# nonl4331/raytracing-rust

Measured on AMD Instinct MI355X. Metric: Msamples/s on rtweekend1.ssml 1920x1080x1024spp, higher is better.
Workload: dtype f32

## Files before the change

include/rt_hip.h:

```cpp
#ifndef RT_HIP_H
#define RT_HIP_H

#include <stdint.h>

#ifdef __cplusplus
extern "C" {
#endif

#define RT_ABI_VERSION 2u

typedef enum rt_status {
	RT_OK = 0,
	RT_ERR_INVALID_ARGUMENT = -1,
	RT_ERR_NO_DEVICE = -2,
	RT_ERR_HIP = -3,
	RT_ERR_OUT_OF_MEMORY = -4,
	RT_ERR_UNSUPPORTED = -5
} rt_status;

typedef enum rt_texture_type {
	RT_TEX_CHECKERED = 0,
	RT_TEX_SOLID = 1,
	RT_TEX_IMAGE = 2,
	RT_TEX_LERP = 3,
// ... 162 lines not shown
#define RT_DEVICE_NONE (-1)
void rt_scene_destroy(rt_scene *scene);

int rt_scene_create_multi(const rt_scene_desc *desc, const int *devices, uint32_t n_devices, rt_scene **out);
int rt_scene_device_count(const rt_scene *scene, uint32_t *n_devices);
typedef enum rt_gather_mode { RT_GATHER_NONE = 0, RT_GATHER_RCCL = 1, RT_GATHER_PEER = 2, RT_GATHER_PEER_STAGED = 3, RT_GATHER_SAME_DEVICE = 4 } rt_gather_mode;
int rt_scene_gather_info(const rt_scene *scene, int *mode, char *note, uint64_t note_capacity);
int rt_rccl_probe(int *usable, char *note, uint64_t note_capacity);
int rt_scene_auto_sample_split(const rt_scene *scene, const rt_render_opts *opts, uint32_t *split);

int rt_scene_counts(const rt_scene *scene, uint64_t *n_nodes, uint64_t *n_primitives, uint64_t *n_lights);
int rt_scene_get_nodes(const rt_scene *scene, rt_bvh_node *out, uint64_t capacity);
int rt_scene_get_primitive_order(const rt_scene *scene, uint64_t *out, uint64_t capacity);
int rt_scene_get_lights(const rt_scene *scene, uint64_t *out, uint64_t capacity);
int rt_scene_wide_info(const rt_scene *scene, uint64_t *n_wide_nodes, uint32_t *root_ref, uint32_t *stack_depth);
int rt_scene_get_wide_nodes(const rt_scene *scene, void *out, uint64_t capacity_nodes);
int rt_scene_get_leaf_boxes(const rt_scene *scene, float *out, uint64_t capacity_slots);
int rt_scene_get_wide_nodes_compact(const rt_scene *scene, void *out, uint64_t capacity_nodes);
int rt_scene_get_leaf_boxes_compact(const rt_scene *scene, float *out, uint64_t capacity_leaves, uint64_t *n_leaves);

typedef struct rt_sky_info {
	uint32_t res_x, res_y;
	uint32_t guide_k;
	uint32_t inv_res_ok;
	float inv_res_x, inv_res_y;
	uint64_t table_bytes;
} rt_sky_info;
int rt_scene_sky_info(const rt_scene *scene, rt_sky_info *info);
int rt_scene_get_sky_tables(const rt_scene *scene, float *row_cdf, uint64_t capacity_rows, float *marginal_cdf, uint64_t capacity_marginal,
                            uint8_t *guide, uint64_t capacity_guide);

int rt_scene_set_traversal(rt_scene *scene, int mode);
typedef enum rt_tuning_key { RT_TUNE_TRAVERSAL = 0, RT_TUNE_FEATURE_SET = 1, RT_TUNE_SCENE_IN_LDS = 2, RT_TUNE_SCHEDULE = 3, RT_TUNE_WALK = 4,
                             RT_TUNE_STACK_CAP = 5, RT_TUNE_EXCHANGE = 6, RT_TUNE_WHOLE_PIXEL_SHARE = 7 } rt_tuning_key;
int rt_scene_set_tuning(rt_scene *scene, int key, int value);
int rt_plan_work_items(const rt_render_opts *opts, uint32_t split, int share, uint64_t resident_waves, uint32_t *whole_claims,
                       uint64_t *n_items);

int rt_render(rt_scene *scene, const rt_camera *camera, const rt_render_opts *opts, float *out_rgb,
              uint64_t *rays_shot);

int rt_render_device(rt_scene *scene, const rt_camera *camera, const rt_render_opts *opts, float *d_out_rgb,
                     uint64_t *d_rays_shot, void *hip_stream);

int rt_render_output_floats(const rt_render_opts *opts, uint64_t *n_floats);
int rt_shard_pixel_order(const rt_render_opts *opts, uint64_t *out, uint64_t capacity);

typedef struct rt_sampler_progress {
	uint64_t samples_completed;
	uint64_t rays_shot;
	const float *current_image;
	uint64_t n_floats;
} rt_sampler_progress;
typedef int (*rt_presentation_update)(void *data, const rt_sampler_progress *progress, uint64_t samples_done);
int rt_sample_image(rt_scene *scene, const rt_camera *camera, const rt_render_opts *opts, uint64_t batch,
                    rt_presentation_update update, void *data);

int rt_last_kernel_ms(rt_scene *scene, float *ms, uint32_t *n_launches);

typedef struct rt_launch_info {
	int32_t method;
	int32_t pruned;
	int32_t fine;
	int32_t sky_in_lds;
	int32_t scene_in_lds;
	int32_t feature_set;
	uint32_t block_threads;
	uint32_t n_blocks;
	uint32_t blocks_per_cu;
	uint32_t waves_per_simd;
	uint32_t lds_bytes;
	uint32_t n_cus;
	uint32_t sample_split;
	uint32_t whole_claims;
	uint64_t n_items;
	char kernel[160];
} rt_launch_info;
int rt_last_launch_info(const rt_scene *scene, rt_launch_info *out);

int rt_output_rgb8(const float *rgb, uint64_t n_values, float gamma, uint8_t *out);
int rt_output_save(const char *filename, const float *rgb, uint32_t width, uint32_t height, float gamma);

int rt_output_rgb8_device(rt_scene *scene, const float *d_rgb, uint64_t n_values, float gamma, uint8_t *d_out, void *hip_stream);
int rt_render_rgb8(rt_scene *scene, const rt_camera *camera, const rt_render_opts *opts, float gamma, uint8_t *out_rgb8,
                   uint64_t *rays_shot);

int rt_check_hit(rt_scene *scene, const rt_ray_desc *rays, uint64_t n_rays, rt_hit_record *out);
int rt_check_hit_index(rt_scene *scene, const rt_ray_desc *rays, const uint64_t *object_index, uint64_t n_rays,
                       rt_hit_record *out);

typedef struct rt_aov_buffers {
	float *albedo;
	float *normal;
	float *depth;
	float *coverage;
	uint32_t *primitive;
	uint32_t *material;
} rt_aov_buffers;
int rt_render_aov(rt_scene *scene, const rt_camera *camera, const rt_render_opts *opts, const rt_aov_buffers *host_out);
int rt_render_aov_device(rt_scene *scene, const rt_camera *camera, const rt_render_opts *opts, const rt_aov_buffers *device_out,
                         void *hip_stream);

typedef struct rt_aov_chain_opts {
	uint32_t max_chain;
	float fuzz_limit;
	uint32_t reserved[6];
} rt_aov_chain_opts;
typedef struct rt_aov_chain_buffers {
// ... 259 lines not shown
```

raytracing-rust_amd/abi.py:

```python
import ctypes as C

RT_ABI_VERSION = 2
RT_GATHER_NONE, RT_GATHER_RCCL, RT_GATHER_PEER, RT_GATHER_PEER_STAGED, RT_GATHER_SAME_DEVICE = 0, 1, 2, 3, 4

RT_OK = 0
RT_ERR_INVALID_ARGUMENT = -1
RT_ERR_NO_DEVICE = -2
RT_ERR_HIP = -3
RT_ERR_OUT_OF_MEMORY = -4
RT_ERR_UNSUPPORTED = -5

RT_TEX_CHECKERED, RT_TEX_SOLID, RT_TEX_IMAGE, RT_TEX_LERP, RT_TEX_PERLIN = range(5)
RT_MAT_EMIT, RT_MAT_LAMBERTIAN, RT_MAT_TROWBRIDGE_REITZ, RT_MAT_REFLECT, RT_MAT_REFRACT = range(5)
RT_PRIM_SPHERE, RT_PRIM_TRIANGLE, RT_PRIM_MESH_TRIANGLE = range(3)
RT_SPLIT_SAH, RT_SPLIT_MIDDLE, RT_SPLIT_EQUAL_COUNTS = range(3)
RT_METHOD_NAIVE, RT_METHOD_MIS = range(2)
RT_LAYOUT_FRAME, RT_LAYOUT_SHARD = range(2)
RT_TUNE_TRAVERSAL, RT_TUNE_FEATURE_SET, RT_TUNE_SCENE_IN_LDS, RT_TUNE_SCHEDULE, RT_TUNE_WALK, RT_TUNE_STACK_CAP, RT_TUNE_EXCHANGE, RT_TUNE_WHOLE_PIXEL_SHARE = range(8)

NO_INDEX = 0xFFFFFFFFFFFFFFFF
RT_DEVICE_NONE = -1

f32x3 = C.c_float * 3


class TextureDesc(C.Structure):
    _fields_ = [
        ("type", C.c_int32),
        ("colour_one", f32x3),
        ("colour_two", f32x3),
        ("image_rgb", C.POINTER(C.c_float)),
        ("image_width", C.c_uint32),
        ("image_height", C.c_uint32),
        ("perlin_ran_vecs", C.POINTER(C.c_float)),
        ("perlin_perm", C.POINTER(C.c_uint32)),
    ]


class MaterialDesc(C.Structure):
    _fields_ = [
        ("type", C.c_int32),
        ("texture", C.c_uint32),
        ("param", C.c_float),
        ("ior", f32x3),
        ("metallic", C.c_float),
    ]


class _Sphere(C.Structure):
    _fields_ = [("centre", f32x3), ("radius", C.c_float)]

# ... 103 lines not shown
        ("max", f32x3),
        ("children", C.c_int64 * 2),
        ("primitive_offset", C.c_uint64),
        ("number_primitives", C.c_uint64),
    ]


class SamplerProgressC(C.Structure):
    _fields_ = [
        ("samples_completed", C.c_uint64),
        ("rays_shot", C.c_uint64),
        ("current_image", C.POINTER(C.c_float)),
        ("n_floats", C.c_uint64),
    ]


class LaunchInfo(C.Structure):
    _fields_ = [
        ("method", C.c_int32),
        ("pruned", C.c_int32),
        ("fine", C.c_int32),
        ("sky_in_lds", C.c_int32),
        ("scene_in_lds", C.c_int32),
        ("feature_set", C.c_int32),
        ("block_threads", C.c_uint32),
        ("n_blocks", C.c_uint32),
        ("blocks_per_cu", C.c_uint32),
        ("waves_per_simd", C.c_uint32),
        ("lds_bytes", C.c_uint32),
        ("n_cus", C.c_uint32),
        ("sample_split", C.c_uint32),
        ("whole_claims", C.c_uint32),
        ("n_items", C.c_uint64),
        ("kernel", C.c_char * 160),
    ]


class SkyInfo(C.Structure):
    _fields_ = [
        ("res_x", C.c_uint32),
        ("res_y", C.c_uint32),
        ("guide_k", C.c_uint32),
        ("inv_res_ok", C.c_uint32),
        ("inv_res_x", C.c_float),
        ("inv_res_y", C.c_float),
        ("table_bytes", C.c_uint64),
    ]


class AovBuffers(C.Structure):
    _fields_ = [
        ("albedo", C.POINTER(C.c_float)),
        ("normal", C.POINTER(C.c_float)),
        ("depth", C.POINTER(C.c_float)),
        ("coverage", C.POINTER(C.c_float)),
        ("primitive", C.POINTER(C.c_uint32)),
        ("material", C.POINTER(C.c_uint32)),
    ]


AOV_CHANNELS = ("albedo", "normal", "depth", "coverage", "primitive", "material")


class AovChainOpts(C.Structure):
    _fields_ = [
        ("max_chain", C.c_uint32),
# ... 265 lines not shown
        ("sigma_normal", C.c_float),
        ("depth_tolerance", C.c_float),
        ("reserved", C.c_uint32 * 8),
    ]


UPSCALE_INPUTS = ("color", "src_albedo", "src_normal", "src_depth", "dst_albedo", "dst_normal", "dst_depth")
UPSCALE_GUIDES = ("albedo", "normal", "depth")
UPSCALE_OPTIONS = ("sigma_normal", "depth_tolerance")


class UpscaleInputs(C.Structure):
    _fields_ = [(name, C.POINTER(C.c_float)) for name in UPSCALE_INPUTS]


DISPLAY_OPTIONS = tuple(n for n, _ in DisplayOpts._fields_ if n not in ("width", "height", "reserved"))

PresentationUpdate = C.CFUNCTYPE(C.c_int, C.c_void_p, C.POINTER(SamplerProgressC), C.c_uint64)

EXPECTED_SIZES = {
    "rt_texture_desc": (TextureDesc, 64),
    "rt_material_desc": (MaterialDesc, 28),
    "rt_primitive_desc": (PrimitiveDesc, 40),
    "rt_triangle_data": (TriangleData, 72),
    "rt_mesh_desc": (MeshDesc, 32),
    "rt_sky_desc": (SkyDesc, 16),
    "rt_scene_desc": (SceneDesc, 96),
    "rt_camera": (Camera, 48),
    "rt_render_opts": (RenderOpts, 80),
    "rt_hit_record": (HitRecord, 72),
    "rt_ray_desc": (RayDesc, 24),
    "rt_bvh_node": (BvhNode, 56),
    "rt_sampler_progress": (SamplerProgressC, 32),
    "rt_launch_info": (LaunchInfo, 224),
    "rt_sky_info": (SkyInfo, 32),
    "rt_aov_buffers": (AovBuffers, 48),
    "rt_aov_chain_opts": (AovChainOpts, 32),
    "rt_aov_chain_buffers": (AovChainBuffers, 56),
    "rt_matte_opts": (MatteOpts, 32),
    "rt_matte_buffers": (MatteBuffers, 24),
    "rt_ao_opts": (AoOpts, 32),
    "rt_ao_buffers": (AoBuffers, 16),
    "rt_noise_opts": (NoiseOpts, 32),
    "rt_noise_summary": (NoiseSummary, 16),
    "rt_noise_buffers": (NoiseBuffers, 40),
    "rt_noise_result": (NoiseResult, 40),
    "rt_robust_opts": (RobustOpts, 32),
    "rt_robust_buffers": (RobustBuffers, 40),
    "rt_denoise_opts": (DenoiseOpts, 48),
    "rt_denoise_inputs": (DenoiseInputs, 40),
    "rt_temporal_opts": (TemporalOpts, 96),
    "rt_temporal_inputs": (TemporalInputs, 32),
    "rt_display_opts": (DisplayOpts, 104),
    "rt_display_state": (DisplayState, 16),
    "rt_bloom_opts": (BloomOpts, 64),
    "rt_dof_opts": (DofOpts, 64),
    "rt_upscale_opts": (UpscaleOpts, 56),
    "rt_upscale_inputs": (UpscaleInputs, 56),
}

EXPORTED_SYMBOLS = [
    "rt_last_error",
    "rt_abi_version",
    "rt_device_count",
    "rt_render_opts_default",
    "rt_camera_new",
    "rt_scene_create",
# ... 150 lines not shown
```

raytracing-rust_amd/csrc/rt_api.cpp:

```cpp
#include <hip/hip_runtime.h>

#include <cstdio>
#include <cstdlib>
#include <algorithm>
#include <cmath>
#include <cstring>
#include <string>
#include <vector>

#include "../../include/rt_hip.h"
#include "../../include/rt_detmath.h"
#include <dlfcn.h>
#include "rt_api_internal.h"
#include "rt_render.h"

using namespace rt;

thread_local std::string g_error;

constexpr uint32_t kFineAboveTriangles = 4096;
constexpr uint32_t kFineAboveSpheres = 32768;

struct RcclApi {
	void *lib = nullptr;
// ... 607 lines not shown
{
	switch (key) {
	case RT_TUNE_TRAVERSAL:
		return rt_scene_set_traversal(s, value);
	case RT_TUNE_FEATURE_SET:
		if (value < s->min_feature_set || value > 2)
			return fail(RT_ERR_INVALID_ARGUMENT, "feature set must be between the scene's own and 2");
		s->feature_set = value;
		s->feature_set_forced = true;
		return RT_OK;
	case RT_TUNE_SCHEDULE:
		if (value < -1 || value > 1)
			return fail(RT_ERR_INVALID_ARGUMENT, "schedule must be -1, 0 or 1");
		s->schedule_mode = value;
		return RT_OK;
	case RT_TUNE_SCENE_IN_LDS:
		s->scene_lds_allowed = value != 0;
		return RT_OK;
	case RT_TUNE_STACK_CAP:
		if (value < 0 || value > 96)
			return fail(RT_ERR_INVALID_ARGUMENT, "stack cap must be 0 (automatic) or 1..96 entries");
		s->stack_cap_override = (uint32_t)value;
		return RT_OK;
	case RT_TUNE_EXCHANGE:
		if (value < 0 || value > 1)
			return fail(RT_ERR_INVALID_ARGUMENT, "exchange must be 0 (off) or 1 (on where the kernel has it)");
		s->exchange_mode = value;
		return RT_OK;
	case RT_TUNE_WHOLE_PIXEL_SHARE:
		if (value < -1 || value > 16)
			return fail(RT_ERR_INVALID_ARGUMENT, "whole-pixel share must be -1 (automatic) or 0..16 (sixteenths of a shard's tiles)");
		s->whole_share = value;
		return RT_OK;
	case RT_TUNE_WALK:
		if (value < 0 || value > 1)
			return fail(RT_ERR_INVALID_ARGUMENT, "walk must be 0 (automatic) or 1 (two-child walk for every ray)");
		s->dev.narrow_only = (uint32_t)value;
		return RT_OK;
	default:
		return fail(RT_ERR_INVALID_ARGUMENT, "unknown tuning key");
	}
}

int rt_scene_counts(const rt_scene *s, uint64_t *n_nodes, uint64_t *n_primitives, uint64_t *n_lights)
{
	if (!s)
		return fail(RT_ERR_INVALID_ARGUMENT, "null scene");
	if (n_nodes) *n_nodes = s->host.nodes.size();
	if (n_primitives) *n_primitives = s->host.primitive_order.size();
	if (n_lights) *n_lights = s->host.lights.size();
	return RT_OK;
}
int rt_scene_get_nodes(const rt_scene *s, rt_bvh_node *out, uint64_t capacity)
{
	if (!s || !out || capacity < s->host.nodes.size())
		return fail(RT_ERR_INVALID_ARGUMENT, "bad arguments");
	for (size_t i = 0; i < s->host.nodes.size(); ++i) {
		const HostNode &n = s->host.nodes[i];
		std::memcpy(out[i].min, n.min, 12);
		std::memcpy(out[i].max, n.max, 12);
		out[i].children[0] = n.child[0];
		out[i].children[1] = n.child[1];
		out[i].primitive_offset = n.primitive_offset;
		out[i].number_primitives = n.number_primitives;
	}
	return RT_OK;
// ... 183 lines not shown

static void fill_tiling(DevRenderParams &P, const rt_render_opts *o, const ShardGeometry &g)
{
	P.width = (uint32_t)o->width;
	P.height = (uint32_t)o->height;
	P.shard_index = o->shard_index;
	P.shard_count = o->shard_count;
	P.tile_w = g.tile_w;
	P.tile_h = g.tile_h;
	P.tiles_x = g.tiles_x;
	P.tiles_y = g.tiles_y;
	P.n_work = (uint32_t)g.n_work;
}

static uint32_t tiled_order_log2(const rt_render_opts *o, const ShardGeometry &g, uint32_t split)
{
	if (g.tile_w * g.tile_h == 64u && (g.tile_w & (g.tile_w - 1u)) == 0u && o->width < 65536u && o->height < 65536u &&
	    (split & (split - 1u)) == 0u && split <= 64u)
		for (uint32_t lw = 0; lw < 7u; ++lw)
			for (uint32_t ls = 0; ls < 7u; ++ls)
				if ((1u << lw) == g.tile_w && (1u << ls) == split)
					return lw | (ls << 8);
	return 0xFFFFFFFFu;
}

struct RenderLaunchPlan {
	DevRenderParams P;
	DevScene dev;
	bool prune, fine, sky_lds, scene_lds, xchg;
	int feature_set, blocks_per_cu;
	uint32_t block_threads, n_blocks;
	size_t lds_bytes;
	uint32_t split;
};

static int plan_render_launch(const rt_scene *s, const rt_render_opts *o, const ShardGeometry &g, RenderLaunchPlan *plan)
{
	DevRenderParams P;
	std::memset(&P, 0, sizeof P);
	fill_tiling(P, o, g);
	P.spp = (uint32_t)o->samples_per_pixel;
	P.sample_begin_lo = (uint32_t)o->sample_begin;
	P.sample_begin_hi = (uint32_t)(o->sample_begin >> 32);
	P.seed_lo = (uint32_t)o->seed;
	P.seed_hi = (uint32_t)(o->seed >> 32);
	P.max_depth = o->max_depth;
	P.rr_threshold = o->rr_threshold;
	uint32_t split = o->sample_split;
	if (split == 0u)
		split = auto_sample_split(s->n_cus, o->width * o->height, o->samples_per_pixel, o->shard_count);
	{
		float rw = 0.0f, rh = 0.0f;
		const bool sized = o->width <= (1u << 24) && o->height <= (1u << 24);
		const bool ok_w = sized && verified_reciprocal((float)(o->width - 1), &rw), ok_h = sized && verified_reciprocal((float)(o->height - 1), &rh);
		const bool ok = ok_w && ok_h;
		P.w1h1_ok = ok ? 1u : 0u;
		P.inv_w1 = rw;
		P.inv_h1 = rh;
	}
	P.tile_log2_w = tiled_order_log2(o, g, split);
	if (split > o->samples_per_pixel)
		return fail(RT_ERR_INVALID_ARGUMENT, "sample_split larger than samples_per_pixel");
	if (g.n_work * split >= (1ull << 32))
		return fail(RT_ERR_UNSUPPORTED, "pixels x sample_split exceeds 2^32 work items");
	P.sample_split = split;
	P.shard_layout = o->output_layout == RT_LAYOUT_SHARD ? 1 : 0;
// ... 83 lines not shown
	if (blocks_per_cu < 1)
		return fail(RT_ERR_HIP, "render kernel does not fit on a CU");
	P.xchg_slots = 0;
	if (xchg && !fine) {
		int blocks_plain = 0;
		if (render_occupancy(o->render_method, prune, fine, sky_lds, feature_set, lds_bytes, &blocks_plain, true) != hipSuccess || blocks_plain < 1) {
			xchg = false;
		} else {
			const int target = std::min(blocks_per_cu, blocks_plain);
			const size_t share = s->max_lds / (size_t)target;
			uint32_t slots = render_exchange_max_slots();
			while (slots >= 16u && lds_bytes + render_exchange_lds_bytes(slots) > share)
				slots -= 4u;
			int blocks_x = 0;
			if (slots >= 16u &&
			    render_occupancy(o->render_method, prune, fine, sky_lds, feature_set, lds_bytes + render_exchange_lds_bytes(slots), &blocks_x, true) == hipSuccess &&
			    blocks_x >= target) {
				P.xchg_slots = slots;
				lds_bytes += render_exchange_lds_bytes(slots);
				blocks_per_cu = target;
			} else {
				xchg = false;
			}
		}
	}
	uint64_t n_blocks = (uint64_t)s->n_cus * (uint64_t)blocks_per_cu;
	const WorkItems items = plan_work_items(g.n_tiles_owned, (uint64_t)g.tile_w * g.tile_h, split, P.tile_log2_w != 0xFFFFFFFFu,
	                                        feature_set == 3 ? s->whole_share : 0, n_blocks * (block_threads / 64u));
	P.whole_claims = (uint32_t)items.whole_claims;
	P.n_items = (uint32_t)items.n_items;
	const uint64_t blocks_needed = ((uint64_t)P.n_items + block_threads - 1) / block_threads;
	if (n_blocks > blocks_needed)
		n_blocks = blocks_needed ? blocks_needed : 1;
	*plan = {P, dev, prune, fine, sky_lds, scene_lds, xchg, feature_set, blocks_per_cu, block_threads, (uint32_t)n_blocks, lds_bytes, split};
	return RT_OK;
}

static void fill_launch_info(const RenderLaunchPlan &plan, const rt_render_opts *o, int n_cus, rt_launch_info *out)
{
	rt_launch_info &L = *out;
	std::memset(&L, 0, sizeof L);
	L.method = o->render_method;
	L.pruned = plan.prune ? 1 : 0;
	L.fine = plan.fine ? 1 : 0;
	L.sky_in_lds = plan.sky_lds ? 1 : 0;
	L.scene_in_lds = plan.scene_lds ? 1 : 0;
	L.feature_set = plan.feature_set;
	L.block_threads = plan.block_threads;
	L.n_blocks = plan.n_blocks;
	L.blocks_per_cu = (uint32_t)plan.blocks_per_cu;
	L.waves_per_simd = (uint32_t)plan.blocks_per_cu * L.block_threads / 256u;
	L.lds_bytes = (uint32_t)plan.lds_bytes;
	L.n_cus = (uint32_t)n_cus;
	L.sample_split = plan.split;
	L.whole_claims = plan.P.whole_claims;
	L.n_items = plan.P.n_items;
	static const char *const feat_names[4] = {"rt::Feat<false, false, false, false>", "rt::Feat<true, true, false, false>",
	                                          "rt::Feat<true, true, true, true>", "rt::FeatPair"};
	std::snprintf(L.kernel, sizeof L.kernel, "rt::render_kernel<%d, %s, %s, %s, %s%s>", (int)o->render_method, plan.prune ? "true" : "false",
	              plan.fine ? "true" : "false", (plan.sky_lds && o->render_method == RT_METHOD_MIS) ? "true" : "false", feat_names[plan.feature_set],
	              plan.xchg ? ", true" : ", false");
}

extern "C" {

int rt_scene_auto_sample_split(const rt_scene *s, const rt_render_opts *o, uint32_t *split)
{
	if (!s || !o || !split)
		return fail(RT_ERR_INVALID_ARGUMENT, "null argument");
	if (s->device == RT_DEVICE_NONE)
		return fail(RT_ERR_NO_DEVICE, "host-only scene (RT_DEVICE_NONE): the split depends on the device's size");
	if (o->shard_count == 0 || o->samples_per_pixel == 0)
		return fail(RT_ERR_INVALID_ARGUMENT, "shard_count and samples_per_pixel must be >= 1");
	const uint32_t members = (uint32_t)(1 + s->peers.size());
	*split = auto_sample_split(s->n_cus, o->width * o->height, o->samples_per_pixel, members > 1u ? members : o->shard_count);
	return RT_OK;
}

int rt_plan_work_items(const rt_render_opts *o, uint32_t split, int share, uint64_t resident_waves, uint32_t *whole_claims, uint64_t *n_items)
{
	ShardGeometry g;
	int rc = shard_geometry(o, g);
	if (rc != RT_OK)
		return rc;
	if (!whole_claims || !n_items)
		return fail(RT_ERR_INVALID_ARGUMENT, "null argument");
	if (split == 0u || share < -1 || share > 16)
		return fail(RT_ERR_INVALID_ARGUMENT, "split must be >= 1 (explicit) and the whole-pixel share -1 (automatic) or 0..16");
	if (g.n_work * split >= (1ull << 32))
// ... 221 lines not shown
		return rc;
	const DevRenderParams &P = plan.P;
	float *render_target = d_out_rgb;
	if (plan.split > 1u) {
		const size_t need = (size_t)g.n_work * plan.split * 3;
		rc = grow_device_buffer(s->d_partial, s->partial_floats, need);
		if (rc != RT_OK)
			return rc;
		render_target = s->d_partial;
	}
	if (P.stack_ovf_depth != 0u) {
		const size_t need = (size_t)plan.n_blocks * plan.block_threads * P.stack_ovf_depth;
		rc = grow_device_buffer(s->d_stack_ovf, s->stack_ovf_words, need);
		if (rc != RT_OK)
			return rc;
	}
	{
		size_t zero_floats = 0;
		if (o->output_layout == RT_LAYOUT_FRAME && o->shard_count > 1)
			zero_floats = (size_t)(o->width * o->height * 3);
		if (o->output_layout == RT_LAYOUT_SHARD)
			zero_floats = (size_t)(g.n_work * 3);
		HIP_TRY(launch_reset(stream, s->d_work_counter, reinterpret_cast<unsigned long long *>(d_rays_shot), d_out_rgb, zero_floats));
	}
	fill_launch_info(plan, o, s->n_cus, &s->last_launch);
	DevCamera cam;
	std::memcpy(cam.origin, camera->origin, 12);
	std::memcpy(cam.lower_left, camera->lower_left, 12);
	std::memcpy(cam.horizontal, camera->horizontal, 12);
	std::memcpy(cam.vertical, camera->vertical, 12);
	DevPairPrimary primary{};
	if (plan.feature_set == 3)
		pair_primary_terms(s->pair, plan.dev.root_min, plan.dev.root_max, v3(cam.origin[0], cam.origin[1], cam.origin[2]), primary);
	HIP_TRY(hipEventRecord(s->ev_start, stream));
	HIP_TRY(launch_render(o->render_method, plan.prune, plan.fine, plan.sky_lds, plan.feature_set, plan.n_blocks, plan.lds_bytes, stream, plan.dev, cam, P,
	                      render_target, reinterpret_cast<unsigned long long *>(d_rays_shot), s->d_work_counter, s->d_stack_ovf, plan.xchg,
	                      plan.feature_set == 3 ? &s->pair : nullptr, plan.feature_set == 3 ? &primary : nullptr, plan.block_threads));
	HIP_TRY(hipEventRecord(s->ev_stop, stream));
	if (plan.split > 1u)
		HIP_TRY(launch_combine(stream, P, s->d_partial, d_out_rgb));
	s->timed = true;
	s->n_launches = 1;
	return RT_OK;
}

int rt_render(rt_scene *s, const rt_camera *camera, const rt_render_opts *o, float *out_rgb, uint64_t *rays_shot)
{
	if (!s || !camera || !o)
		return fail(RT_ERR_INVALID_ARGUMENT, "null argument");
	if (int rc = need_device(s); rc != RT_OK)
		return rc;
	uint64_t n_floats = 0;
	int rc = rt_render_output_floats(o, &n_floats);
	if (rc != RT_OK)
		return rc;
	if (n_floats == 0) {
		if (rays_shot)
			*rays_shot = 0;
		return RT_OK;
	}
	if (!out_rgb)
		return fail(RT_ERR_INVALID_ARGUMENT, "null argument");
	HIP_TRY(hipSetDevice(s->device));
	rc = ensure_frame_buffers(s, n_floats, false);
	if (rc != RT_OK)
		return rc;
// ... 170 lines not shown
```

raytracing-rust_amd/csrc/rt_api_internal.h:

```cpp
#pragma once
#include <hip/hip_runtime.h>

#include <cstdint>
#include <string>
#include <vector>

#include "../../include/rt_hip.h"
#include "rt_build.h"
#include "rt_types.h"

extern thread_local std::string g_error;

inline int fail(int code, const std::string &msg)
{
	g_error = msg;
	return code;
}
inline int hip_fail(hipError_t e, const char *what)
{
	g_error = std::string(what) + ": " + hipGetErrorString(e);
	return e == hipErrorOutOfMemory ? RT_ERR_OUT_OF_MEMORY : RT_ERR_HIP;
}
#define HIP_TRY(expr)                       \
	do {                                    \
// ... 9 lines not shown
struct rt_scene {
	int device = 0;
	rt::HostScene host;
	rt::DevScene dev{};
	std::vector<void *> allocations;
	hipStream_t stream = nullptr;
	uint32_t *d_work_counter = nullptr;
	unsigned long long *d_rays = nullptr;
	hipEvent_t ev_start = nullptr, ev_stop = nullptr;
	bool timed = false;
	uint32_t n_launches = 0;
	int n_cus = 0;
	int traversal_mode = -1;
	int schedule_mode = -1;
	int feature_set = 2;
	int min_feature_set = 0;
	bool pair_tree = false, feature_set_forced = false;
	rt::DevPairScene pair{};
	bool scene_lds_allowed = true;
	float *d_partial = nullptr;
	size_t partial_floats = 0;
	float *d_prog[2] = {nullptr, nullptr};
	float *h_prog[2] = {nullptr, nullptr};
	unsigned long long *d_prog_rays = nullptr;
	unsigned long long *h_prog_rays = nullptr;
	size_t d_prog_floats[2] = {0, 0}, h_prog_floats[2] = {0, 0};
	hipStream_t copy_stream = nullptr;
	hipEvent_t ev_batch[2] = {nullptr, nullptr}, ev_copy[2] = {nullptr, nullptr};
	size_t max_lds = 65536;
	rt_launch_info last_launch{};
	uint32_t stack_cap_override = 0;
	int exchange_mode = 0;
	int whole_share = kWholeShareDefault;
	uint32_t stack_depth_narrow = 2;
	uint32_t *d_stack_ovf = nullptr;
	size_t stack_ovf_words = 0;
	uint8_t *d_rgb8 = nullptr;
	size_t d_rgb8_bytes = 0;
	std::vector<rt_scene *> peers;
	bool member_call = false;
	float *d_shard = nullptr;
	size_t shard_floats = 0;
	unsigned long long *d_member_rays = nullptr;
	hipEvent_t ev_shard = nullptr;
	hipEvent_t ev_begin = nullptr;
	float *d_gather = nullptr;
	size_t gather_floats = 0;
	unsigned long long *d_gather_rays = nullptr;
	void *nccl_comms = nullptr;
	int gather_mode = 0;
	std::string gather_note;
	hipEvent_t ev_gathered = nullptr;
	bool gathered_once = false;
	uint32_t *d_prim_desc = nullptr;
	char *d_denoise = nullptr;
	size_t d_denoise_bytes = 0;
	char *d_temporal = nullptr;
	uint32_t temporal_w = 0, temporal_h = 0;
	int temporal_cur = -1;
	rt_camera temporal_prev{};
	char *d_display = nullptr;
	size_t d_display_bytes = 0;
	uint32_t display_w = 0, display_h = 0;
	bool display_has_state = false;
	char *d_noise = nullptr;
	size_t d_noise_bytes = 0;
// ... 148 lines not shown
```

raytracing-rust_amd/csrc/rt_render.h:

```cpp
#pragma once
#include <hip/hip_runtime.h>
#include "rt_types.h"

namespace rt {
size_t render_lds_bytes(const DevScene &S, bool sky_lds, bool scene_lds, uint32_t waves_per_block, uint32_t stack_cap);
uint32_t render_waves_per_simd(int feature_set, bool fine);
uint32_t render_block_threads(int feature_set, bool fine, bool xchg = false);
uint32_t render_max_block_threads(int feature_set, bool fine, bool xchg);
hipError_t render_occupancy(int method, bool prune, bool fine, bool sky_lds, int feature_set, size_t lds_bytes, int *blocks_per_cu, bool xchg,
                            uint32_t block_threads = 0);
bool render_exchange_available(int method, bool prune, bool fine, int feature_set);
size_t render_exchange_lds_bytes(uint32_t slots);
uint32_t render_exchange_max_slots();
size_t render_exchange_fine_lds_bytes(uint32_t waves_per_block);

hipError_t launch_reset(hipStream_t stream, uint32_t *work_counter, unsigned long long *rays_shot, float *out, size_t n_out_floats);
hipError_t launch_render(int method, bool prune, bool fine, bool sky_lds, int feature_set, uint32_t n_blocks, size_t lds_bytes, hipStream_t stream,
                         const DevScene &S, const DevCamera &cam, const DevRenderParams &P, float *out,
                         unsigned long long *rays_shot, uint32_t *work_counter, uint32_t *stack_ovf, bool xchg, const DevPairScene *pair,
                         const DevPairPrimary *primary, uint32_t block_threads = 0);
hipError_t launch_combine(hipStream_t stream, const DevRenderParams &P, const float *partial, float *out);
hipError_t launch_scatter_shard(hipStream_t stream, const DevRenderParams &P, const float *shard, float *frame);
hipError_t launch_sum_u64(hipStream_t stream, const unsigned long long *parts, uint32_t n, unsigned long long *out);
hipError_t launch_quantise(hipStream_t stream, const float *rgb, size_t n_values, float inv_gamma, uint8_t *out);
}
```

raytracing-rust_amd/csrc/rt_render.hip:

```cpp
#include "rt_shade.h"
#include "rt_render.h"

namespace rt {

enum : int {
	PH_GEN = 0,
	PH_NODE = 1,
	PH_LEAF = 2,
	PH_SHADE = 3,
	PH_LIGHT = 4,
	PH_SCATTER = 5,
	PH_NARROW = 6,
	PH_COUNT = 7,
	PH_NEED_PIXEL = 7,
	PH_DONE = 8,
	PH_WALK = 9
};

#ifndef RT_PQ_SPLIT
#define RT_PQ_SPLIT 1
#endif
#ifndef RT_LIGHT_PHASE_THRESHOLD
#define RT_LIGHT_PHASE_THRESHOLD 48
#endif
constexpr uint32_t kLightPhaseThreshold = RT_LIGHT_PHASE_THRESHOLD;
#ifndef RT_STARVE_LIMIT
#define RT_STARVE_LIMIT 128
#endif
constexpr uint32_t kStarveLimit = RT_STARVE_LIMIT;
constexpr uint32_t kClaim = 64;
constexpr uint32_t kWholePixel = 64u;
constexpr uint32_t kWholeClaim = 1u << 31;
#ifndef RT_ACQUIRE_BATCH
#define RT_ACQUIRE_BATCH 1
#endif
constexpr uint32_t kAcquireBatch = RT_ACQUIRE_BATCH;
#ifndef RT_FULL_WAVES
#define RT_FULL_WAVES 5
#endif
#ifndef RT_FULL_FINE_WAVES
#define RT_FULL_FINE_WAVES 4
#endif
#ifndef RT_SIMPLE_FINE_WAVES
#define RT_SIMPLE_FINE_WAVES 4
#endif
#ifndef RT_SIMPLE_COARSE_WAVES
#define RT_SIMPLE_COARSE_WAVES 5
#endif
#ifndef RT_SIMPLE_COARSE_BLOCK
#define RT_SIMPLE_COARSE_BLOCK 256
#endif
#ifndef RT_SPHERES_BLOCK
#define RT_SPHERES_BLOCK 512
#endif
#ifndef RT_FUSE_REGIONS
#define RT_FUSE_REGIONS(spheres_only) true
#endif
#ifndef RT_BODY_ALWAYS
#define RT_BODY_ALWAYS(spheres_only) true
#endif
#ifndef RT_SPHERES_MAX_BLOCK
#define RT_SPHERES_MAX_BLOCK 768
#endif
#ifndef RT_PAIR_WAVES
#define RT_PAIR_WAVES 6
#endif
#ifndef RT_SPHERES_WAVES
#define RT_SPHERES_WAVES 4
#endif
// ... 177 lines not shown
		const char *b = reinterpret_cast<const char *>(lds_blob);
		S.nodes = reinterpret_cast<const DevNode *>(b + S.off_nodes);
		S.prims = reinterpret_cast<const DevPrim *>(b + S.off_prims);
		S.shade = reinterpret_cast<const DevShade *>(b + S.off_shade);
		S.prim_rank = reinterpret_cast<const uint32_t *>(b + S.off_rank);
		S.materials = reinterpret_cast<const DevMaterial *>(b + S.off_materials);
		S.textures = reinterpret_cast<const DevTexture *>(b + S.off_textures);
		S.lights = reinterpret_cast<const uint32_t *>(b + S.off_lights);
		S.big_leaves = reinterpret_cast<const uint2 *>(b + S.off_big_leaves);
	}
	StackMem SM;
	SM.cap = P.stack_cap;
	SM.ovf_depth = P.stack_ovf_depth;
	SM.ovf = stack_ovf;
	SM.region = lds + sky_words + blob_words;
	uint32_t *stk = SM.region + wave * (P.stack_cap * kStackStride) + lane;
	uint32_t *pool = nullptr;
	if constexpr (XCHG) {
		pool = lds + (((uint32_t)(SM.region - lds) + (blockDim.x >> 6) * (P.stack_cap * kStackStride) + 3u) & ~3u);
		if (FINE) {
			if (threadIdx.x < kXchgFineHdr)
				pool[threadIdx.x] = threadIdx.x == 3u ? kXchgShaderWaves : (threadIdx.x == 4u ? (blockDim.x >> 6) - kXchgShaderWaves : 0u);
		} else if (threadIdx.x < 4u) {
			pool[threadIdx.x] = 0u;
		}
		__syncthreads();
	}

#ifdef RT_STATS
	unsigned long long st_iters[2] = {0, 0}, st_active[2] = {0, 0}, st_gen = 0, st_hist[8] = {};
	unsigned long long st_sect[16] = {}, st_mark = wall_clock64();
	unsigned long long st_fine_clock[PH_COUNT + 1] = {};
	unsigned long long st_fine_iters[PH_COUNT] = {}, st_fine_active[PH_COUNT] = {};
#endif
	const bool sky_samplable = sky_can_sample(S);
	constexpr bool kWholeItems = F::pair && !FINE;
	static_assert(!(kWholeItems && XCHG), "the exchange's records carry chunk_begin and chunk_end, not chunk_c: no whole-pixel items there");
	constexpr int known_path = F::known_materials ? kMatLambertian : kMatRead;

	int ph = PH_NEED_PIXEL;
	rt_rng rng = {1u, 2u, 3u, 4u};
	Ray ray;
	ray.o = ray.d = ray.inv = ray.shear = v3s(0.0f);
	uint32_t node = kRefDone;
	int sp = 0;
	float best_t = 0.0f;
	uint32_t best_prim = kNoPrim;
	bool any_hit = false;
	V3 thr = v3s(1.0f), outp = v3s(0.0f), mean = v3s(0.0f), wo = v3s(0.0f);
	Hit hit;
	hit.t = 0.0f;
	hit.point = hit.error = hit.normal = v3s(0.0f);
	hit.err_dot = 0.0f;
	hit.uvx = hit.uvy = 0.0f;
	hit.has_uv = hit.out = false;
	uint32_t mat = 0;
	uint32_t depth = 0, out_index = 0, pixel_index = 0, px = 0, py = 0;
	uint32_t sample_i = 0, chunk_begin = 0, chunk_end = P.spp, chunk_c = 0;
	uint32_t ray_count = 0;
	unsigned long long rays_total = 0;
	bool primary = true;
	struct LightCtx {
		V3 l_wi;
		float pdf_multiplier;
		float t_limit;
		uint32_t skip;
// ... 1005 lines not shown
			constexpr bool kBodyAlways = RT_BODY_ALWAYS(KernelShape<F>::spheres_only);
			if (kBodyAlways) {
				alive = (n_light + n_trace != 0u) || __ballot(ph == PH_NEED_PIXEL) != 0ull;
				if (XCHG && METHOD == 1 && !alive)
					alive = __hip_atomic_load(&pool[1], __ATOMIC_RELAXED, __HIP_MEMORY_SCOPE_WORKGROUP) != 0u ||
					        __hip_atomic_load(&pool[2], __ATOMIC_RELAXED, __HIP_MEMORY_SCOPE_WORKGROUP) != 0u;
			}
			if (kBodyAlways || n_light + n_trace != 0u) {
				const bool run_light = (METHOD == 1) && (n_light >= kLightPhaseThreshold || n_trace == 0u || (kStarveLimit != 0u && waited >= kStarveLimit));
				waited = run_light ? 0u : waited + n_light;
	#ifdef RT_STATS
				if (lane == 0u) {
					if (!run_light) {
						st_iters[0] += 1; st_active[0] += n_trace;
						st_hist[((n_trace ? n_trace : 1u) - 1u) >> 3] += 1;
#ifndef RT_STATS_NO_HIST
						atomicAdd(&g_hist[0][n_trace], 1ull);
						atomicAdd(&g_hist[1][n_light], 1ull);
#endif
						st_gen += (unsigned long long)__popcll(__ballot(ph == PH_GEN));
					} else {
						st_iters[1] += 1; st_active[1] += n_light;
#ifndef RT_STATS_NO_HIST
						atomicAdd(&g_hist[3][n_light], 1ull);
#endif
					}
				}
	#endif
				RT_SECTION(0);
				constexpr bool kFuseRegions = METHOD == 1 && RT_PQ_SPLIT && RT_FUSE_REGIONS(KernelShape<F>::spheres_only);
				bool run_q = run_light;
				if (!run_light) {
					if (kFuseRegions) {
						if (ph == PH_GEN) {
							load_pair_scene(std::false_type{});
							do_gen();
							load_pair_primary();
							RT_SECTION(1);
							walk_closest_primary();
							RT_SECTION(2);
							do_shade(std::integral_constant<int, 1>{});
						}
						RT_SECTION(3);
						const uint32_t n_light_now = (uint32_t)__popcll(__ballot(ph == PH_LIGHT));
						run_q = n_light_now >= kLightPhaseThreshold;
						if (run_q)
							waited = 0u;
	#ifdef RT_STATS
						if (run_q && lane == 0u) {
							st_iters[1] += 1; st_active[1] += n_light_now;
						}
	#endif
					} else {
						load_pair_scene(std::true_type{});
						if (ph == PH_GEN)
							do_gen();
						RT_SECTION(1);
						walk_closest_pending();
						RT_SECTION(2);
						if (ph == PH_SHADE)
							do_shade(std::integral_constant<int, (METHOD == 1 && RT_PQ_SPLIT) ? 1 : 0>{});
						RT_SECTION(3);
					}
				}
				if (run_q) {
					LightCtx L;
					L.l_wi = v3s(0.0f);
					L.pdf_multiplier = 1.0f;
					L.t_limit = 0.0f;
					L.skip = kNoPrim;
					L.have_shadow = L.shadow_is_sky = false;
					Ray sray;
					sray.o = sray.d = sray.inv = sray.shear = v3s(0.0f);
					if (kFuseRegions) {
						if (ph == PH_LIGHT) {
							load_pair_scene(std::true_type{});
							do_light(L, sray);
// ... 33 lines not shown
					ray.o = ray.d = ray.inv = ray.shear = v3s(0.0f);
					best_t = 0.0f;
					best_prim = kNoPrim;
					node = kRefDone;
					sp = 0;
					any_hit = false;
				}
	#endif
			} else {
				alive = __ballot(ph == PH_NEED_PIXEL) != 0ull;
				if (XCHG && METHOD == 1)
					alive = alive || __hip_atomic_load(&pool[1], __ATOMIC_RELAXED, __HIP_MEMORY_SCOPE_WORKGROUP) != 0u ||
					        __hip_atomic_load(&pool[2], __ATOMIC_RELAXED, __HIP_MEMORY_SCOPE_WORKGROUP) != 0u;
			}
		}
	}
#ifdef RT_STATS
	atomicAdd(&g_stats[20], st_lane_nodes);
	atomicAdd(&g_stats[21], st_lane_prims);
	atomicMax(&g_stats[22], st_lane_maxsp);
	if (lane == 0u) {
		for (int k = 0; k < 9; ++k)
			atomicAdd(&g_stats[40 + k], st_sect[k]);
		if (!FINE)
			for (int k = 9; k < 16; ++k)
				atomicAdd(&g_stats[40 + k], st_sect[k]);
		for (int k = 0; k < 8; ++k)
			atomicAdd(&g_stats[24 + k], st_hist[k]);
		for (int k = 0; k <= PH_COUNT; ++k)
			atomicAdd(&g_stats[50 + k], st_fine_clock[k]);
		atomicAdd(&g_stats[0], st_iters[0]); atomicAdd(&g_stats[1], st_active[0]);
		atomicAdd(&g_stats[2], st_iters[1]); atomicAdd(&g_stats[3], st_active[1]);
		atomicAdd(&g_stats[4], st_gen);
		for (int k = 0; k < PH_COUNT; ++k) {
			atomicAdd(&g_stats[5 + k], st_fine_iters[k]);
			atomicAdd(&g_stats[5 + PH_COUNT + k], st_fine_active[k]);
		}
	}
#endif
	unsigned long long *const rays_shot = K->rays_shot;
	if (rays_shot != nullptr) {
		for (int off = 32; off > 0; off >>= 1)
			rays_total += __shfl_down(rays_total, off);
		if (lane == 0u)
			atomicAdd(rays_shot, rays_total);
	}
}

__global__ __launch_bounds__(256) void combine_chunks_kernel(const DevRenderParams P, const float *__restrict__ partial, float *__restrict__ out)
{
	const uint32_t wp = blockIdx.x * blockDim.x + threadIdx.x;
	if (wp >= P.n_work)
		return;
	uint32_t x, y;
	if (!work_to_pixel(P, wp, x, y))
		return;
	V3 acc = v3s(0.0f);
	for (uint32_t c = 0; c < P.sample_split; ++c) {
		const float *m = partial + 3u * ((size_t)c * P.n_work + wp);
		acc.x = acc.x + m[0];
		acc.y = acc.y + m[1];
		acc.z = acc.z + m[2];
	}
	const size_t o = P.shard_layout ? (size_t)wp : (size_t)y * P.width + x;
	out[3u * o + 0u] = acc.x / (float)P.spp;
	out[3u * o + 1u] = acc.y / (float)P.spp;
// ... 88 lines not shown
{
	hipLaunchKernelGGL(sum_u64_kernel, dim3(1), dim3(1), 0, stream, parts, n, out);
	return hipGetLastError();
}

hipError_t launch_combine(hipStream_t stream, const DevRenderParams &P, const float *partial, float *out)
{
	hipLaunchKernelGGL(combine_chunks_kernel, dim3((P.n_work + 255u) / 256u), dim3(256), 0, stream, P, partial, out);
	return hipGetLastError();
}

#ifdef RT_STATS
extern "C" int rt_debug_hist(unsigned long long *out260, int reset)
{
	if (hipMemcpyFromSymbol(out260, HIP_SYMBOL(g_hist), sizeof(g_hist)) != hipSuccess)
		return -1;
	if (reset) {
		unsigned long long z[4 * 65] = {};
		(void)hipMemcpyToSymbol(HIP_SYMBOL(g_hist), z, sizeof z);
	}
	return 0;
}
extern "C" int rt_debug_stats(unsigned long long *out16, int reset)
{
	if (hipMemcpyFromSymbol(out16, HIP_SYMBOL(g_stats), sizeof(g_stats)) != hipSuccess)
		return -1;
	if (reset) {
		unsigned long long z[64] = {};
		(void)hipMemcpyToSymbol(HIP_SYMBOL(g_stats), z, sizeof z);
	}
	return 0;
}
#endif

uint32_t render_block_threads(int feature_set, bool fine, bool xchg)
{
	if (fine && xchg)
		return 512u;
	if (feature_set == 3)
		return (uint32_t)KernelShape<FeatPair>::block;
	if (feature_set == 0)
		return (uint32_t)KernelShape<Feat<false, false, false, false>>::block;
	if (feature_set == 1)
		return fine ? (uint32_t)KernelShape<Feat<true, true, false, false>, true>::block : (uint32_t)KernelShape<Feat<true, true, false, false>, false>::block;
	return 256u;
}

uint32_t render_max_block_threads(int feature_set, bool fine, bool xchg)
{
	if (fine || xchg)
		return render_block_threads(feature_set, fine, xchg);
	if (feature_set == 3)
		return (uint32_t)KernelShape<FeatPair>::max_block;
	if (feature_set == 0)
		return (uint32_t)KernelShape<Feat<false, false, false, false>>::max_block;
	if (feature_set == 1)
		return (uint32_t)KernelShape<Feat<true, true, false, false>>::max_block;
	return render_block_threads(feature_set, fine, xchg);
}

uint32_t render_waves_per_simd(int feature_set, bool fine)
{
	if (feature_set == 3)
		return (uint32_t)KernelShape<FeatPair>::waves_per_simd;
	if (feature_set == 0)
		return fine ? (uint32_t)KernelShape<Feat<false, false, false, false>, true>::waves_per_simd : (uint32_t)KernelShape<Feat<false, false, false, false>, false>::waves_per_simd;
// ... 124 lines not shown
```

raytracing-rust_amd/csrc/rt_types.h:

```cpp
#pragma once

#include <stdint.h>
#include "rt_vec.h"

namespace rt {

constexpr uint32_t kNoPrim = 0xFFFFFFFFu;

template <bool TRI, bool LIGHTS, bool CMAT, bool CTEX> struct Feat {
	static constexpr bool tri = TRI;
	static constexpr bool lights = LIGHTS;
	static constexpr bool cmat = CMAT;
	static constexpr bool ctex = CTEX;
	static constexpr bool pair = false;
	static constexpr bool known_materials = false;
};
using FeatFull = Feat<true, true, true, true>;
struct FeatPair : Feat<false, false, false, false> {
	static constexpr bool pair = true;
	static constexpr bool known_materials = true;
};

constexpr uint32_t kLeafFlag = 0x80000000u;
constexpr uint32_t kLeafInlineMax = 31u;
// ... 98 lines not shown
	const DevLeafBox *leaf_box;
	uint32_t root4_ref;
	uint32_t n_nodes4;
	uint32_t narrow_only;
	uint32_t has_triangles;
	uint32_t lambert_tame;
	uint32_t single_light;
	DevSky sky;
};

constexpr int kStackStride = 64;
constexpr uint32_t kFourWaves = 4;
inline size_t four_wave_stack_lds_bytes(const DevScene &S) { return (size_t)kFourWaves * S.stack_depth * kStackStride * sizeof(uint32_t); }

struct alignas(64) DevPairScene {
	float c0min[3], c0max[3], c1min[3], c1max[3];
	uint32_t slot0, slot1;
	uint32_t rank0, rank1;
	float sphere[2][4];
	float lambert[2][4];
	float sky_param;
	int32_t sky_tex_type;
	float sky_c1[3], sky_c2[3];
	float inv_radius[2];
	uint32_t pad[6];
};
static_assert(sizeof(DevPairScene) == 192, "DevPairScene: three 64-byte lines");
__device__ static const DevPairScene kNoPairScene = {};

struct alignas(64) DevPairPrimary {
	float box[2][2][3];
	float sphere[2][4];
	uint32_t valid;
	float deltapdot[2];
	float root[2][3];
	uint32_t pad[3];
};
static_assert(sizeof(DevPairPrimary) == 128, "DevPairPrimary: two 64-byte lines");
constexpr int kPairPrimaryValues = 28;
RT_FN void pair_primary_terms(const DevPairScene &q, const float root_min[3], const float root_max[3], V3 o, DevPairPrimary &pp)
{
	const float oc[3] = {o.x, o.y, o.z};
	bool finite = finite_f(o.x) && finite_f(o.y) && finite_f(o.z);
	for (int k = 0; k < 3; ++k) {
		pp.box[0][0][k] = q.c0min[k] - oc[k]; pp.box[0][1][k] = q.c0max[k] - oc[k];
		pp.box[1][0][k] = q.c1min[k] - oc[k]; pp.box[1][1][k] = q.c1max[k] - oc[k];
		pp.root[0][k] = root_min[k] - oc[k]; pp.root[1][k] = root_max[k] - oc[k];
		finite = finite && finite_f(pp.box[0][0][k]) && finite_f(pp.box[0][1][k]) && finite_f(pp.box[1][0][k]) && finite_f(pp.box[1][1][k]) &&
		         finite_f(pp.root[0][k]) && finite_f(pp.root[1][k]);
	}
	for (int s = 0; s < 2; ++s) {
		const float radius = q.sphere[s][3];
		const V3 deltap = v3(q.sphere[s][0], q.sphere[s][1], q.sphere[s][2]) - o;
		const float deltapdot = dot(deltap, deltap);
		pp.sphere[s][0] = deltap.x; pp.sphere[s][1] = deltap.y; pp.sphere[s][2] = deltap.z;
		pp.deltapdot[s] = deltapdot;
		pp.sphere[s][3] = deltapdot - radius * radius;
		finite = finite && finite_f(deltap.x) && finite_f(deltap.y) && finite_f(deltap.z) && finite_f(deltapdot) && finite_f(pp.sphere[s][3]);
	}
	pp.valid = finite ? 1u : 0u;
	pp.pad[0] = pp.pad[1] = pp.pad[2] = 0u;
}

struct DevCamera {
	float origin[3], lower_left[3], horizontal[3], vertical[3];
};

struct DevRenderParams {
	uint32_t width, height;
	uint32_t spp;
	uint32_t sample_begin_lo, sample_begin_hi;
	uint32_t seed_lo, seed_hi;
	uint32_t max_depth, rr_threshold;
	uint32_t shard_index, shard_count;
	uint32_t tile_w, tile_h, tiles_x, tiles_y;
	uint32_t n_work;
	uint32_t sample_split;
	uint32_t n_items;
	int32_t shard_layout;
	int32_t prune;
	uint32_t sky_in_lds;
	uint32_t scene_in_lds;
	uint32_t stack_cap;
	uint32_t stack_ovf_depth;
	uint32_t xchg_slots;
	uint32_t tile_log2_w;
	uint32_t whole_claims;
	uint32_t w1h1_ok;
	float inv_w1, inv_h1;
};

}
```

Measured before the change: 37870.

## Add tunable primary-ray run loop repeating gen passes before light phase

Adds a tunable 'primary run' cap that lets a wave repeat the generate/primary-walk/shade step several times while few lanes are waiting in the light phase. The aim is to keep lanes busy with primary rays instead of falling through to scheduling overhead. Extra wave ballots are computed each pass, and the pair-scene load is moved out of the per-lane generate branch. The default compile-time cap is 1, so repetition is effectively off unless tuned. A launch-info field and a tuning key are added to expose the setting.

```diff
diff --git a/include/rt_hip.h b/include/rt_hip.h
--- a/include/rt_hip.h
+++ b/include/rt_hip.h
@@ -218,7 +218,7 @@
 
 int rt_scene_set_traversal(rt_scene *scene, int mode);
 typedef enum rt_tuning_key { RT_TUNE_TRAVERSAL = 0, RT_TUNE_FEATURE_SET = 1, RT_TUNE_SCENE_IN_LDS = 2, RT_TUNE_SCHEDULE = 3, RT_TUNE_WALK = 4,
-                             RT_TUNE_STACK_CAP = 5, RT_TUNE_EXCHANGE = 6, RT_TUNE_WHOLE_PIXEL_SHARE = 7 } rt_tuning_key;
+                             RT_TUNE_STACK_CAP = 5, RT_TUNE_EXCHANGE = 6, RT_TUNE_WHOLE_PIXEL_SHARE = 7, RT_TUNE_PRIMARY_RUN = 8 } rt_tuning_key;
 int rt_scene_set_tuning(rt_scene *scene, int key, int value);
 int rt_plan_work_items(const rt_render_opts *opts, uint32_t split, int share, uint64_t resident_waves, uint32_t *whole_claims,
                        uint64_t *n_items);
@@ -260,6 +260,8 @@
 	uint32_t sample_split;
 	uint32_t whole_claims;
 	uint64_t n_items;
+	uint32_t primary_run;
+	uint32_t reserved;
 	char kernel[160];
 } rt_launch_info;
 int rt_last_launch_info(const rt_scene *scene, rt_launch_info *out);
diff --git a/raytracing-rust_amd/abi.py b/raytracing-rust_amd/abi.py
--- a/raytracing-rust_amd/abi.py
+++ b/raytracing-rust_amd/abi.py
@@ -16,7 +16,7 @@
 RT_SPLIT_SAH, RT_SPLIT_MIDDLE, RT_SPLIT_EQUAL_COUNTS = range(3)
 RT_METHOD_NAIVE, RT_METHOD_MIS = range(2)
 RT_LAYOUT_FRAME, RT_LAYOUT_SHARD = range(2)
-RT_TUNE_TRAVERSAL, RT_TUNE_FEATURE_SET, RT_TUNE_SCENE_IN_LDS, RT_TUNE_SCHEDULE, RT_TUNE_WALK, RT_TUNE_STACK_CAP, RT_TUNE_EXCHANGE, RT_TUNE_WHOLE_PIXEL_SHARE = range(8)
+RT_TUNE_TRAVERSAL, RT_TUNE_FEATURE_SET, RT_TUNE_SCENE_IN_LDS, RT_TUNE_SCHEDULE, RT_TUNE_WALK, RT_TUNE_STACK_CAP, RT_TUNE_EXCHANGE, RT_TUNE_WHOLE_PIXEL_SHARE, RT_TUNE_PRIMARY_RUN = range(9)
 
 NO_INDEX = 0xFFFFFFFFFFFFFFFF
 RT_DEVICE_NONE = -1
@@ -186,6 +186,8 @@
         ("sample_split", C.c_uint32),
         ("whole_claims", C.c_uint32),
         ("n_items", C.c_uint64),
+        ("primary_run", C.c_uint32),
+        ("reserved", C.c_uint32),
         ("kernel", C.c_char * 160),
     ]
 
@@ -517,7 +519,7 @@
     "rt_ray_desc": (RayDesc, 24),
     "rt_bvh_node": (BvhNode, 56),
     "rt_sampler_progress": (SamplerProgressC, 32),
-    "rt_launch_info": (LaunchInfo, 224),
+    "rt_launch_info": (LaunchInfo, 232),
     "rt_sky_info": (SkyInfo, 32),
     "rt_aov_buffers": (AovBuffers, 48),
     "rt_aov_chain_opts": (AovChainOpts, 32),
diff --git a/raytracing-rust_amd/csrc/rt_api.cpp b/raytracing-rust_amd/csrc/rt_api.cpp
--- a/raytracing-rust_amd/csrc/rt_api.cpp
+++ b/raytracing-rust_amd/csrc/rt_api.cpp
@@ -663,6 +663,11 @@
 			return fail(RT_ERR_INVALID_ARGUMENT, "whole-pixel share must be -1 (automatic) or 0..16 (sixteenths of a shard's tiles)");
 		s->whole_share = value;
 		return RT_OK;
+	case RT_TUNE_PRIMARY_RUN:
+		if (value < 0 || (uint32_t)value > kPrimaryRunMax)
+			return fail(RT_ERR_INVALID_ARGUMENT, "primary run must be 0 (automatic), 1 (off) or a cap of 2..32767 passes");
+		s->primary_run = (uint32_t)value;
+		return RT_OK;
 	case RT_TUNE_WALK:
 		if (value < 0 || value > 1)
 			return fail(RT_ERR_INVALID_ARGUMENT, "walk must be 0 (automatic) or 1 (two-child walk for every ray)");
@@ -912,6 +917,7 @@
 	uint32_t block_threads, n_blocks;
 	size_t lds_bytes;
 	uint32_t split;
+	uint32_t primary_run;
 };
 
 static int plan_render_launch(const rt_scene *s, const rt_render_opts *o, const ShardGeometry &g, RenderLaunchPlan *plan)
@@ -1061,7 +1067,8 @@
 	const uint64_t blocks_needed = ((uint64_t)P.n_items + block_threads - 1) / block_threads;
 	if (n_blocks > blocks_needed)
 		n_blocks = blocks_needed ? blocks_needed : 1;
-	*plan = {P, dev, prune, fine, sky_lds, scene_lds, xchg, feature_set, blocks_per_cu, block_threads, (uint32_t)n_blocks, lds_bytes, split};
+	const uint32_t primary_run = (feature_set == 3 && o->render_method == RT_METHOD_MIS) ? (s->primary_run ? s->primary_run : render_primary_run_default()) : 1u;
+	*plan = {P, dev, prune, fine, sky_lds, scene_lds, xchg, feature_set, blocks_per_cu, block_threads, (uint32_t)n_blocks, lds_bytes, split, primary_run};
 	return RT_OK;
 }
 
@@ -1084,6 +1091,7 @@
 	L.sample_split = plan.split;
 	L.whole_claims = plan.P.whole_claims;
 	L.n_items = plan.P.n_items;
+	L.primary_run = plan.primary_run;
 	static const char *const feat_names[4] = {"rt::Feat<false, false, false, false>", "rt::Feat<true, true, false, false>",
 	                                          "rt::Feat<true, true, true, true>", "rt::FeatPair"};
 	std::snprintf(L.kernel, sizeof L.kernel, "rt::render_kernel<%d, %s, %s, %s, %s%s>", (int)o->render_method, plan.prune ? "true" : "false",
@@ -1371,6 +1379,7 @@
 	DevPairPrimary primary{};
 	if (plan.feature_set == 3)
 		pair_primary_terms(s->pair, plan.dev.root_min, plan.dev.root_max, v3(cam.origin[0], cam.origin[1], cam.origin[2]), primary);
+	primary.run = plan.primary_run;
 	HIP_TRY(hipEventRecord(s->ev_start, stream));
 	HIP_TRY(launch_render(o->render_method, plan.prune, plan.fine, plan.sky_lds, plan.feature_set, plan.n_blocks, plan.lds_bytes, stream, plan.dev, cam, P,
 	                      render_target, reinterpret_cast<unsigned long long *>(d_rays_shot), s->d_work_counter, s->d_stack_ovf, plan.xchg,
diff --git a/raytracing-rust_amd/csrc/rt_api_internal.h b/raytracing-rust_amd/csrc/rt_api_internal.h
--- a/raytracing-rust_amd/csrc/rt_api_internal.h
+++ b/raytracing-rust_amd/csrc/rt_api_internal.h
@@ -65,6 +65,7 @@
 	uint32_t stack_cap_override = 0;
 	int exchange_mode = 0;
 	int whole_share = kWholeShareDefault;
+	uint32_t primary_run = 0;
 	uint32_t stack_depth_narrow = 2;
 	uint32_t *d_stack_ovf = nullptr;
 	size_t stack_ovf_words = 0;
diff --git a/raytracing-rust_amd/csrc/rt_render.h b/raytracing-rust_amd/csrc/rt_render.h
--- a/raytracing-rust_amd/csrc/rt_render.h
+++ b/raytracing-rust_amd/csrc/rt_render.h
@@ -6,6 +6,8 @@
 size_t render_lds_bytes(const DevScene &S, bool sky_lds, bool scene_lds, uint32_t waves_per_block, uint32_t stack_cap);
 uint32_t render_waves_per_simd(int feature_set, bool fine);
 uint32_t render_block_threads(int feature_set, bool fine, bool xchg = false);
+uint32_t render_primary_run_default();
+constexpr uint32_t kPrimaryRunMax = 32767;
 uint32_t render_max_block_threads(int feature_set, bool fine, bool xchg);
 hipError_t render_occupancy(int method, bool prune, bool fine, bool sky_lds, int feature_set, size_t lds_bytes, int *blocks_per_cu, bool xchg,
                             uint32_t block_threads = 0);
diff --git a/raytracing-rust_amd/csrc/rt_render.hip b/raytracing-rust_amd/csrc/rt_render.hip
--- a/raytracing-rust_amd/csrc/rt_render.hip
+++ b/raytracing-rust_amd/csrc/rt_render.hip
@@ -35,6 +35,11 @@
 #define RT_ACQUIRE_BATCH 1
 #endif
 constexpr uint32_t kAcquireBatch = RT_ACQUIRE_BATCH;
+#ifndef RT_PRIMARY_RUN
+#define RT_PRIMARY_RUN 1
+#endif
+static_assert(RT_PRIMARY_RUN >= 1, "RT_PRIMARY_RUN: 1 = off, n = cap");
+constexpr uint32_t kPrimaryRunDefault = RT_PRIMARY_RUN;
 #ifndef RT_FULL_WAVES
 #define RT_FULL_WAVES 5
 #endif
@@ -278,6 +283,7 @@
 	unsigned long long st_sect[16] = {}, st_mark = wall_clock64();
 	unsigned long long st_fine_clock[PH_COUNT + 1] = {};
 	unsigned long long st_fine_iters[PH_COUNT] = {}, st_fine_active[PH_COUNT] = {};
+	unsigned long long st_run[3] = {};
 #endif
 	const bool sky_samplable = sky_can_sample(S);
 	constexpr bool kWholeItems = F::pair && !FINE;
@@ -1349,17 +1355,55 @@
 				bool run_q = run_light;
 				if (!run_light) {
 					if (kFuseRegions) {
-						if (ph == PH_GEN) {
+						constexpr bool kPrimaryRun = F::pair && !XCHG;
+						uint32_t n_light_now;
+						if constexpr (kPrimaryRun) {
 							load_pair_scene(std::false_type{});
-							do_gen();
-							load_pair_primary();
-							RT_SECTION(1);
-							walk_closest_primary();
-							RT_SECTION(2);
-							do_shade(std::integral_constant<int, 1>{});
+							bool again;
+							do {
+								if (ph == PH_GEN) {
+									do_gen();
+									load_pair_primary();
+									RT_SECTION(1);
+									walk_closest_primary();
+									RT_SECTION(2);
+									do_shade(std::integral_constant<int, 1>{});
+								}
+								RT_SECTION(3);
+								n_light_now = (uint32_t)__popcll(__ballot(ph == PH_LIGHT));
+								const uint32_t n_gen_now = (uint32_t)__popcll(__ballot(ph == PH_GEN));
+								const bool repeatable = __ballot(ph == PH_NEED_PIXEL) == 0ull && n_gen_now != 0u && n_light_now < kLightPhaseThreshold &&
+								                        (kStarveLimit == 0u || (waited & 0xFFFFu) + n_light_now < kStarveLimit);
+								again = repeatable && (waited >> 16) + 1u < K->primary.run;
+	#ifdef RT_STATS
+								if (lane == 0u) {
+									st_run[0] += repeatable ? 1u : 0u;
+									st_run[1] += 1;
+									st_run[2] += again ? 1u : 0u;
+									if (again) {
+										st_iters[0] += 1; st_active[0] += n_gen_now;
+										st_hist[(n_gen_now - 1u) >> 3] += 1;
+										st_gen += n_gen_now;
+									}
+								}
+	#endif
+								if (again)
+									waited += n_light_now + 0x10000u;
+							} while (__builtin_expect(again, false));
+							waited &= 0xFFFFu;
+						} else {
+							if (ph == PH_GEN) {
+								load_pair_scene(std::false_type{});
+								do_gen();
+								load_pair_primary();
+								RT_SECTION(1);
+								walk_closest_primary();
+								RT_SECTION(2);
+								do_shade(std::integral_constant<int, 1>{});
+							}
+							RT_SECTION(3);
+							n_light_now = (uint32_t)__popcll(__ballot(ph == PH_LIGHT));
 						}
-						RT_SECTION(3);
-						const uint32_t n_light_now = (uint32_t)__popcll(__ballot(ph == PH_LIGHT));
 						run_q = n_light_now >= kLightPhaseThreshold;
 						if (run_q)
 							waited = 0u;
@@ -1459,6 +1503,8 @@
 		atomicAdd(&g_stats[0], st_iters[0]); atomicAdd(&g_stats[1], st_active[0]);
 		atomicAdd(&g_stats[2], st_iters[1]); atomicAdd(&g_stats[3], st_active[1]);
 		atomicAdd(&g_stats[4], st_gen);
+		for (int k = 0; k < 3; ++k)
+			atomicAdd(&g_stats[32 + k], st_run[k]);
 		for (int k = 0; k < PH_COUNT; ++k) {
 			atomicAdd(&g_stats[5 + k], st_fine_iters[k]);
 			atomicAdd(&g_stats[5 + PH_COUNT + k], st_fine_active[k]);
@@ -1613,6 +1659,8 @@
 	return 0;
 }
 #endif
+
+uint32_t render_primary_run_default() { return kPrimaryRunDefault; }
 
 uint32_t render_block_threads(int feature_set, bool fine, bool xchg)
 {
diff --git a/raytracing-rust_amd/csrc/rt_types.h b/raytracing-rust_amd/csrc/rt_types.h
--- a/raytracing-rust_amd/csrc/rt_types.h
+++ b/raytracing-rust_amd/csrc/rt_types.h
@@ -154,9 +154,10 @@
 	float box[2][2][3];
 	float sphere[2][4];
 	uint32_t valid;
+	uint32_t run;
 	float deltapdot[2];
 	float root[2][3];
-	uint32_t pad[3];
+	uint32_t pad[2];
 };
 static_assert(sizeof(DevPairPrimary) == 128, "DevPairPrimary: two 64-byte lines");
 constexpr int kPairPrimaryValues = 28;
@@ -181,7 +182,8 @@
 		finite = finite && finite_f(deltap.x) && finite_f(deltap.y) && finite_f(deltap.z) && finite_f(deltapdot) && finite_f(pp.sphere[s][3]);
 	}
 	pp.valid = finite ? 1u : 0u;
-	pp.pad[0] = pp.pad[1] = pp.pad[2] = 0u;
+	pp.run = 1u;
+	pp.pad[0] = pp.pad[1] = 0u;
 }
 
 struct DevCamera {
```

Measured after the change: 37690. No clear change (-0.5%).
